# MPEGGroup/mpeg-pcc-tmc13

Measured on AMD Instinct MI355X. Metric: RAHT forward+inverse attribute-transform Mpoints/s (bit-exact vs CPU reference), higher is better.
Workload: dtype int64 (Q15 fixed point), int32 I/O; 1 GPU; subnode=1 pred=1 ext=1 qp34: RAHT forward+inverse, 1x1000000 Morton-sorted S-lidar/GPU, C=1; frames_per_gpu=1, roundtrip_decoder_equals_encoder_recon=True

## Files before the change

### mpeg-pcc-tmc13_amd/csrc/gpcc_attr_mi355.hip

```cpp
#include <hip/hip_runtime.h>

#include <algorithm>
#include <cstdio>
#include <cstdlib>
#include <dlfcn.h>
#include <cstring>
#include <atomic>
#include <deque>
#include <map>
#include <mutex>
#include <thread>
#include <string>
#include <cmath>
#include <vector>

#include "gpcc_attr_mi355.h"
#include "raht_common.hpp"
#include "raht_edges.hpp"
#include "raht_levels.hpp"
#include "raht_rdoq.hpp"
#include "raht_subnode.hpp"
#include "raht_pipe.hpp"
#include "raht_sweep.hpp"
#include "raht_tile.hpp"
// ... 960 lines not shown
    rc.state = pl.rtile_state;
    rc.c = C;
    HIP_TRY(hipMemsetAsync(pl.rtile_state, 0, ((size_t)pl.num_rtiles + 1) * sizeof(unsigned long long), st));
    HIP_TRY(hipMemsetAsync(pl.slice_l, 0xff, 2 * (size_t)s * sizeof(int32_t), st));
  }

  if (tiles) {
    lc.li = 0;
    const int cgrid = std::min(s, 2048);
    if (!encoder) {
      Timer t(ctx, "coarse_synth");
      raht_coarse_kernel<C, kCoarseDecode><<<cgrid, 1024, 0, st>>>(lc);
    } else if (pl.haar) {
      Timer t(ctx, "coarse_fused");
      raht_coarse_kernel<C, kCoarseHaar><<<cgrid, 1024, 0, st>>>(lc);
    } else {
      Timer t(ctx, "coarse_lossy");
      raht_coarse_kernel<C, kCoarseLossy><<<cgrid, 1024, 0, st>>>(lc);
    }
  }

  HIP_TRY(hipEventSynchronize(ctx->ev_stats));
  const TreeStats ts = *ctx->h_stats;
  const int first_level = std::min(nlev - 1, tiles ? ts.fine_levels : ts.max_top);

  bool piped = false;
  if (pl.pipe && first_level >= 1) {
    PipeCtx px{};
    int64_t total = 0;
    for (int li = 0; li <= first_level; li++) {
      px.uoff[li] = (int32_t)total;
      total += ts.nodes[li];
    }
    const size_t need = (size_t)total * (4 + 1 + 4 + 32 * C) + 2048;
    void* pipe_mem = nullptr;
    PoolScope pipe_pool(ctx);
    if (total * C * 16 < ((int64_t)1 << 31) && pipe_pool.take_bytes(need, &pipe_mem) == hipSuccess) {
      Arena pa;
      pa.base = (char*)pipe_mem;
      pa.cap = need;
      px.g = pa.take<uint32_t>((size_t)total * C * 4);
      px.u = pa.take<uint32_t>((size_t)total * C * 4);
      px.src = pa.take<int32_t>(total);
      px.worklist = pa.take<int32_t>(total);
      px.pocc = pa.take<uint8_t>(total);
      px.total = (int32_t)total;
      px.top = first_level;
      px.tag = 1;
      px.ticket = lc.ticket;
      HIP_TRY(hipMemsetAsync(px.g, 0, (size_t)total * C * 16, st));
      HIP_TRY(hipMemsetAsync(px.u, 0, (size_t)total * C * 16, st));
      {
        Timer t(ctx, "pipe_prepass");
        pipe_iota_kernel<<<grid_for(total, 256), 256, 0, st>>>(px.src, (int)total);
        for (int li = first_level - 1; li >= 0; li--) {
          lc.li = li;
          const int64_t parents = ts.nodes[li + 1];
          raht_pipe_prepass_kernel<C><<<(int)std::min<int64_t>((parents + 1023) / 1024, 1024), 256, 0, st>>>(lc, px);
        }
      }
      {
        Timer t(ctx, "pipe_synth");
        if (pl.f64)
          raht_pipe_synth_kernel<C, ArithF64><<<kSubGrid, 256, 0, st>>>(lc, px);
        else
          raht_pipe_synth_kernel<C><<<kSubGrid, 256, 0, st>>>(lc, px);
      }
      {
        Timer t(ctx, "pipe_leaf");
        pipe_leaf_kernel<C><<<grid_for(ts.nodes[0], 256), 256, 0, st>>>(lc, px);
      }
      piped = true;
    }
  }

  LinkSchedule links;
  auto link_prof = [&](const char* name, int li) { return Timer(ctx, li < 0 ? name : level_name(name, li)); };
  const bool use_links = pl.links && !piped && !tiles && first_level >= 1 && hp->raht_extension != 0;
  if (use_links) {
    links.tv = tv;
    links.lv = pl.lv;
    links.begin(st, ts.nodes, first_level, link_prof);
  }
  int level_from = first_level;
  static const int rec_mode = [] {
    const char* e = getenv("GPCC_REC");
    return e ? atoi(e) : 0;
  }();
  const bool ext_flag = hp->raht_extension != 0;
  const bool use_rec = pl.sub && !pl.haar && !pl.has_qp && !pl.links && !piped && rec_mode == 1;
  size_t rec_need = 0;
  if (use_rec)
// ... 5888 lines not shown
```

### mpeg-pcc-tmc13_amd/csrc/raht_levels.hpp

```cpp
#pragma once

#include "raht_common.hpp"

namespace gpcc {

enum LevelMode { kAnalyze = 0, kSynth = 1, kFused = 2, kLossySub = 3 };

constexpr uint32_t kDescNever = 0x7fffffffu;
constexpr uint32_t kDescZero = 0x80000000u;

typedef const __attribute__((address_space(4))) gpcc_raht_params* ParamsConst;

struct InterRef {
  const int64_t* pos;
  const int32_t* prefix;
  int32_t n_ref;
  int32_t lr;
  int32_t blocks;
  int32_t dual;
  int32_t filtered;
  const int32_t* tap;
  const int64_t* hkey;
  const int32_t* hfp;
  const int32_t* hlf;
  const int32_t* hsoff;
  uint32_t* idesc;
  int64_t* iptrans;
  int32_t* icoeffs;
};

enum SweepField {
  kSfW = 0, kSfCa = 1, kSfCb = 4, kSfNsq = 7, kSfNrs = 8, kSfPn = 9, kSfNbc0 = 12, kSfPk = 15, kSfPk2 = 16,
  kSfC0 = 17, kSfSlice = 18, kSweepFields = 19
};

struct SweepRec {
  int32_t* f32;
  int64_t* src;
  uint8_t* occ;
  int32_t lanes;
  int32_t rbase[kMaxLevels];
  const int32_t* worklist;
  const int32_t* work_count;
};


struct LevelCtx {
  TreeView tv;
  const gpcc_raht_params* params;
  const SliceSched* sched;
  const int32_t* attr_prefix;
  const int32_t* const* haar_lf;
  const int32_t* const* asc_qp;
  int64_t* rec[2];
  int64_t* rec_us[2];
  int32_t* nneigh[2];
  int32_t* dqp[2];
  int32_t* coeffs;
  uint32_t* desc;
  int64_t* ptrans;
  int32_t li;
  const struct SharedLut* lut;
  int32_t* worklist;
  int32_t* work_count;
  unsigned long long* scan_state;
  uint8_t* pocc;
  uint32_t* mbox;
  uint32_t mtag;
  int32_t* ticket;
  int32_t* error;
  unsigned long long* rdoq_state;
  int32_t* slice_l;
  InterRef inter;
  const int32_t* link_rec;
  const int32_t* link_lrec;
  int32_t claim_rounds;
  SweepRec brec;
};
// ... 332 lines not shown
```

### mpeg-pcc-tmc13_amd/csrc/raht_pipe.hpp

```cpp
#pragma once

#include "raht_arith.hpp"
#include "raht_subnode.hpp"

namespace gpcc {

#ifdef GPCC_PIPE_PROF
__device__ unsigned long long g_pipe_prof[32 * 8];
struct PipeProf {
  unsigned long long last = 0;
  int li = 0;
  __device__ void begin(int l) { li = l; last = __builtin_amdgcn_s_memtime(); }
  __device__ void mark(int stage, int lane)
  {
    const unsigned long long t = __builtin_amdgcn_s_memtime();
    if (lane == 0)
      atomicAdd(&g_pipe_prof[li * 8 + stage], t - last);
    last = t;
  }
  __device__ void round(int lane) { if (lane == 0) atomicAdd(&g_pipe_prof[li * 8 + 7], 1ull); }
};
#else
struct PipeProf {
  __device__ void begin(int) {}
  __device__ void mark(int, int) {}
  __device__ void round(int) {}
};
#endif

struct PipeCtx {
  int32_t* src;
  uint32_t* g;
  uint32_t* u;
  uint8_t* pocc;
  int32_t* worklist;
  int32_t uoff[kMaxLevels + 1];
  int32_t total;
  int32_t top;
  uint32_t tag;
  int32_t* ticket;
};

constexpr int32_t kPipeCopied = (int32_t)0x80000000;
constexpr int32_t kPipeIndex = 0x7fffffff;

__global__ __launch_bounds__(256) void
pipe_iota_kernel(int32_t* src, int n)
{
  for (int i = blockIdx.x * blockDim.x + threadIdx.x; i < n; i += gridDim.x * blockDim.x)
    src[i] = i;
}

template<int C>
__global__ __launch_bounds__(256) void
raht_pipe_prepass_kernel(LevelCtx ctx, PipeCtx px)
{
  __shared__ int wave_cnt[4];
  __shared__ int base_s;
  if (tree_failed(ctx.tv))
    return;
  const TreeView& tv = ctx.tv;
  const int li = ctx.li;
  const bool ext = ctx.params->raht_extension != 0;
  const int num_parents = tv.soff[li + 1][tv.num_slices];
  const int lane = lane_id(), wave = threadIdx.x >> 6;
  const int pbase = px.uoff[li + 1], cbase = px.uoff[li];
  const int64_t chunks = ((int64_t)num_parents + 255) >> 8;
  const int64_t per = (chunks + gridDim.x - 1) / gridDim.x;
  const int64_t gbeg = min((int64_t)blockIdx.x * per, chunks);
  const int64_t gend = min(gbeg + per, chunks);

  int mine = 0;
  for (int64_t chunk = gbeg; chunk < gend; chunk++) {
// ... 78 lines not shown
    int off = running;
    for (int w = 0; w < wave; w++)
      off += wave_cnt[w];
    if (real)
      px.worklist[pbase + off + __popcll(m & ((1ull << lane) - 1))] = j;
    running += wave_cnt[0] + wave_cnt[1] + wave_cnt[2] + wave_cnt[3];
  }
}

template<int C>
__global__ __launch_bounds__(256) void
pipe_leaf_kernel(LevelCtx ctx, PipeCtx px)
{
  if (tree_failed(ctx.tv))
    return;
  const TreeView& tv = ctx.tv;
  const int m = tv.soff[0][tv.num_slices];
  for (int j = blockIdx.x * blockDim.x + threadIdx.x; j < m; j += gridDim.x * blockDim.x) {
    const int s = find_slice(tv.soff[0], tv.num_slices, j);
    const SliceSched* sc = &ctx.sched[s];
    if (sc->num_unique <= 1)
      continue;
    const int64_t row = (int64_t)tv.pt_off[s] + (j - tv.soff[0][s]);
    const int from = px.src[px.uoff[0] + j] & kPipeIndex;
    const u32x4* gp = reinterpret_cast<const u32x4*>(px.g);
#pragma unroll
    for (int k = 0; k < C; k++) {
      const u32x4 gv = gp[(size_t)from * C + k];
      par2(ctx.rec, sc->final_parity)[row * C + k] = (int64_t)(((uint64_t)gv.y << 32) | gv.x);
    }
  }
}

template<int C, class A = ArithI64>
__global__ __launch_bounds__(256, C == 3 ? GPCC_SUB_SYNTH3_WAVES : 4) void
raht_pipe_synth_kernel(LevelCtx ctx, PipeCtx px)
{
  typedef typename A::T VT;
  typedef typename A::Coef VC;
  __shared__ SharedLut lut_s;
  if (tree_failed(ctx.tv))
    return;
  load_lut(&lut_s, ctx.lut);
  const SharedLut& lut = lut_s;

  const TreeView& tv = ctx.tv;
  const ParamsConst prm = (ParamsConst)ctx.params;
  const int t = threadIdx.x & 7;
  const int lane = lane_id();
  const int gbase = threadIdx.x & 56;
  const bool haar = !A::kF64 && prm->integer_haar_enable_flag != 0;
  const bool ext = A::kF64 || prm->raht_extension != 0;
  const int cls = blockIdx.x & 7;
  bool in_range = true;
  const auto grsrc = __builtin_amdgcn_make_buffer_rsrc(
    px.g, 0, (int)((size_t)px.total * C * 16), 0x00020000);
  const auto ursrc = __builtin_amdgcn_make_buffer_rsrc(
    px.u, 0, (int)((size_t)px.total * C * 16), 0x00020000);

  for (;;) {
    int tk = 0;
    if (lane == 0)
      tk = atomicAdd(&px.ticket[cls], 1);
    tk = __shfl(tk, 0);
    const int64_t ground = (int64_t)tk * 8 + cls;
    int li = -1;
    int64_t rbase = 0;
    for (int l = px.top - 1; l >= 0; l--) {
      const int64_t r = ((int64_t)ctx.work_count[l] + 7) >> 3;
      if (ground < rbase + r) {
        li = l;
        break;
      }
      rbase += r;
    }
    if (li < 0)
      break;
    if (__hip_atomic_load(ctx.error, __ATOMIC_RELAXED, __HIP_MEMORY_SCOPE_AGENT))
      break;
    PipeProf prof;
    prof.begin(li);
    prof.round(lane);
    const int num_work = ctx.work_count[li];
    const int wi = (int)((ground - rbase) * 8) + (lane >> 3);
    const bool live = wi < num_work;
    const int pbase = px.uoff[li + 1], cbase = px.uoff[li];
    const int j = live ? px.worklist[pbase + wi] : 0;
    int s = 0;
    LevelSched e;
    e.processed = 0;
    if (live) {
      s = find_slice(tv.soff[li + 1], tv.num_slices, j);
      e = ctx.sched[s].lvl[li];
    }
    const bool on = live && e.processed;
    const int sp0 = on ? tv.soff[li + 1][s] : 0;
    const int sp1 = on ? tv.soff[li + 1][s + 1] : 0;
    const int sc0 = on ? tv.soff[li][s] : 0;
    const int pt0 = on ? tv.pt_off[s] : 0;
    const int n_s = on ? tv.pt_off[s + 1] - pt0 : 0;
    const int c0 = on ? tv.fc[li + 1][j] : 0;
    const int nchild = on ? tv.fc[li + 1][j + 1] - c0 : 0;
    const int pj = j - sp0;

    const int64_t ckey = t < nchild ? tv.key[li][c0 + t] : 0;
    const uint32_t occ = group8_or(t < nchild ? 1u << (int)(ckey & 7) : 0u);
    const bool has = (occ >> t) & 1;
    const int child = c0 + popc32(occ & ((1u << t) - 1));
    int32_t w = 0;
    if (has)
      w = tv.fp[li][child + 1] - tv.fp[li][child];

    prof.mark(0, lane);
    int32_t wl[3], wr[3];
    VC ca[3], cb[3];
    int32_t cw = w;
#pragma unroll
    for (int st = 0; st < 3; st++) {
      const int bit = 1 << st;
      const int32_t pw = lane_xor8(cw, bit);
      const bool left = !(t & bit);
      wl[st] = left ? cw : pw;
      wr[st] = left ? pw : cw;
      int64_t ia = 0, ib = 0;
      if (wl[st] && wr[st]) {
        if (!haar)
          raht_coeffs(wl[st], wr[st], lut, &ia, &ib);
        cw = wl[st] + wr[st];
      } else {
        cw = left ? wl[st] + wr[st] : 0;
      }
      ca[st] = A::coef(ia);
      cb[st] = A::coef(ib);
    }

    const bool inherit_dc = !e.is_root;
    const bool pred_in_level = on && inherit_dc && prm->raht_prediction_enabled_flag != 0;
    bool enable_pred = pred_in_level;
    int neigh_count = 0;
    VT pred[C];
#pragma unroll
    for (int k = 0; k < C; k++)
      pred[k] = A::zero();
    bool want_search = false;
    if (pred_in_level) {
      if (ext && nchild == 1) {
        enable_pred = false;
        neigh_count = 19;
      } else {
        want_search = true;
      }
    }
    const int pbase_j = pbase + j;
    const int psrc_raw = (on && inherit_dc && t == 0) ? px.src[pbase_j] : 0;
    const int psrc = psrc_raw & kPipeIndex;
    int64_t own_v[C], own_us[C];
    int own_nn = 0;
    bool a1_done = false;
    {
      const bool need = on && inherit_dc && t == 0;
      u32x4 a[C], b[C];
#pragma unroll
      for (int k = 0; k < C; k++) {
        own_v[k] = own_us[k] = 0;
        a[k] = b[k] = u32x4{0, 0, 0, 0};
        if (need) {
          a[k] = __builtin_amdgcn_raw_buffer_load_b128(grsrc, (psrc * C + k) * 16, 0,  16);
          b[k] = __builtin_amdgcn_raw_buffer_load_b128(ursrc, (psrc * C + k) * 16, 0,  16);
        }
      }
      bool ok = need;
#pragma unroll
      for (int k = 0; k < C; k++)
        ok = ok && a[k].z == px.tag && b[k].z == px.tag;
      if (ok) {
#pragma unroll
        for (int k = 0; k < C; k++) {
          own_v[k] = (int64_t)(((uint64_t)a[k].y << 32) | a[k].x);
          own_us[k] = (int64_t)(((uint64_t)b[k].y << 32) | b[k].x);
        }
        own_nn = (int)a[0].w;
        a1_done = true;
      }
    }
    {
      const int early = __shfl(a1_done ? ((psrc_raw & kPipeCopied) ? 19 : own_nn) : 1 << 20, gbase);
      if (want_search && early < prm->raht_prediction_threshold0)
        want_search = false;
    }
    int pn[3] = {-1, -1, -1};
    {
      int lo[3] = {0, 0, 0}, hi[3] = {0, 0, 0}, end[3] = {0, 0, 0};
      int64_t want[3] = {0, 0, 0};
      if (want_search) {
        const int64_t cur_pos = tv.key[li + 1][j];
        const uint64_t base = morton3d_add((uint64_t)cur_pos, ~0ull);
        const int64_t range = prm->raht_prediction_search_range;
#pragma unroll
        for (int slot = 0; slot < 3; slot++) {
          const int i = 1 + t + 8 * slot;
          if (i < 19 && (occ & neigh_mask(i))) {
            const int64_t np = (int64_t)morton3d_add(base, neigh_offset(i));
            int64_t d = np - cur_pos;
            if (d >= 0) {
              d = d >= range ? range : d;
              lo[slot] = j;
              end[slot] = (d + 1 < (int64_t)(sp1 - j)) ? j + (int)(d + 1) : sp1;
            } else {
              d = (-d) >= range ? range : -d;
              end[slot] = j;
              lo[slot] = (d < (int64_t)(j - sp0)) ? j - (int)d : sp0;
            }
            hi[slot] = end[slot];
            want[slot] = np;
          }
        }
      }
      const int64_t* __restrict__ pkey = tv.key[li + 1];
      while (__any((lo[0] < hi[0]) | (lo[1] < hi[1]) | (lo[2] < hi[2]))) {
        int mid[3];
        int64_t kv[3];
#pragma unroll
        for (int slot = 0; slot < 3; slot++) {
          mid[slot] = lo[slot] + ((hi[slot] - lo[slot]) >> 1);
          kv[slot] = lo[slot] < hi[slot] ? pkey[mid[slot]] : 0;
        }
#pragma unroll
        for (int slot = 0; slot < 3; slot++) {
          if (lo[slot] < hi[slot]) {
            if (kv[slot] < want[slot])
              lo[slot] = mid[slot] + 1;
            else
              hi[slot] = mid[slot];
          }
        }
      }
#pragma unroll
      for (int slot = 0; slot < 3; slot++) {
        if (lo[slot] < end[slot] && pkey[lo[slot]] == want[slot])
          pn[slot] = lo[slot];
      }
    }

    prof.mark(1, lane);
    const uint32_t present = group8_bits(on && cw != 0) | (on ? 1u : 0u);
    const int spos = (0x74516230u >> (4 * t)) & 7;
    const uint32_t pscan = ((present >> 0) & 1) | (((present >> 4) & 1) << 1)
      | (((present >> 2) & 1) << 2) | (((present >> 1) & 1) << 3)
      | (((present >> 6) & 1) << 4) | (((present >> 5) & 1) << 5)
      | (((present >> 3) & 1) << 6) | (((present >> 7) & 1) << 7);
    const int rank = popc32(pscan & ((1u << spos) - 1));
    const bool coded = on && ((present >> t) & 1) && (t != 0 || !inherit_dc);
    const int cidx = e.coeff_base + (inherit_dc ? (c0 - sc0) - pj + rank - 1 : rank);
    const int32_t* __restrict__ cplane = ctx.coeffs + (size_t)pt0 * C + cidx;
    Quantizer qa[2] = {{1, 1}, {1, 1}};
    if (coded) {
      int ac0 = 0, ac1 = 0;
      if (e.ac_layer < prm->num_ac_qp_layers && t) {
        ac0 = prm->ac_qp_offset[e.ac_layer][t - 1][0];
        ac1 = prm->ac_qp_offset[e.ac_layer][t - 1][1];
      }
      qpset_quantizers(prm, e.qp_layer, ac0, ac1, qa);
    }
    int32_t nrm_sq_i = 0, nrm_rs_i = 0, nrm_shift = 0;
    if (!haar && w > 1) {
      nrm_sq_i = (int32_t)sqrt_weight(w, lut);
      if (w < kSmallN) {
        nrm_rs_i = lut.norm_rs[w];
      } else {
        const uint64_t w64 = (uint64_t)w;
        nrm_shift = w64 > 1024 ? ilog2_u64(w64 - 1) >> 1 : 0;
        nrm_rs_i = (int32_t)(irsqrt(w64, lut.rsqrt) >> (40 - nrm_shift - kFpFrac));
      }
    }
    const VC nrm_sq = A::coef(nrm_sq_i), nrm_rs = A::coef(nrm_rs_i);
    const typename A::Quant qaa[2] = {A::quant(qa[0]), A::quant(qa[1])};
    int32_t qc[C];
#pragma unroll
    for (int k = 0; k < C; k++)
      qc[k] = coded ? cplane[(size_t)k * n_s] : 0;

    int nsrc[3] = {0, 0, 0};
#pragma unroll
    for (int slot = 0; slot < 3; slot++)
      if (pn[slot] >= 0)
        nsrc[slot] = px.src[pbase + pn[slot]] & kPipeIndex;

    prof.mark(2, lane);
    unsigned spins = 0;
    bool failed = false;
    {
      bool need = on && inherit_dc && t == 0 && !a1_done;
      while (__any(need)) {
        u32x4 a[C], b[C];
#pragma unroll
        for (int k = 0; k < C; k++) {
          a[k] = b[k] = u32x4{0, 0, 0, 0};
          if (need) {
            a[k] = __builtin_amdgcn_raw_buffer_load_b128(grsrc, (psrc * C + k) * 16, 0,  16);
            b[k] = __builtin_amdgcn_raw_buffer_load_b128(ursrc, (psrc * C + k) * 16, 0,  16);
          }
        }
        bool ok = need;
#pragma unroll
        for (int k = 0; k < C; k++)
          ok = ok && a[k].z == px.tag && b[k].z == px.tag;
        if (ok) {
#pragma unroll
          for (int k = 0; k < C; k++) {
            own_v[k] = (int64_t)(((uint64_t)a[k].y << 32) | a[k].x);
            own_us[k] = (int64_t)(((uint64_t)b[k].y << 32) | b[k].x);
          }
          own_nn = (int)a[0].w;
          need = false;
        }
        if (!__any(ok)) {
          if (++spins > (1u << 21)) {
            failed = true;
            break;
          }
          __builtin_amdgcn_s_sleep(GPCC_SUB_SLEEP);
        }
      }
    }
    const int pneigh = __shfl((psrc_raw & kPipeCopied) ? 19 : own_nn, gbase);
    bool do_search = false;
    if (pred_in_level && !(ext && nchild == 1)) {
      if (pneigh < prm->raht_prediction_threshold0)
        enable_pred = false;
      else
        do_search = true;
    }
    if (!do_search) {
      pn[0] = pn[1] = pn[2] = -1;
    }
    {
      int found = (pn[0] >= 0) + (pn[1] >= 0) + (pn[2] >= 0);
      found = group8_sum(found);
      if (do_search) {
        neigh_count = found + 1;
        if (neigh_count < prm->raht_prediction_threshold1)
          enable_pred = false;
      }
    }
    const bool run = do_search && enable_pred;

    prof.mark(3, lane);
    int64_t nbv[3][C];
#pragma unroll
    for (int slot = 0; slot < 3; slot++)
#pragma unroll
      for (int k = 0; k < C; k++)
        nbv[slot][k] = 0;
    if (!failed) {
      uint32_t need = 0;
#pragma unroll
      for (int slot = 0; slot < 3; slot++)
        if (run && pn[slot] >= 0)
          need |= 1u << slot;
      while (__any(need != 0)) {
        u32x4 a[3][C];
#pragma unroll
        for (int slot = 0; slot < 3; slot++)
#pragma unroll
          for (int k = 0; k < C; k++) {
            a[slot][k] = u32x4{0, 0, 0, 0};
            if ((need >> slot) & 1)
              a[slot][k] = __builtin_amdgcn_raw_buffer_load_b128(
                grsrc, (nsrc[slot] * C + k) * 16, 0,  16);
          }
        bool any_ok = false;
#pragma unroll
        for (int slot = 0; slot < 3; slot++) {
          bool ok = (need >> slot) & 1;
#pragma unroll
          for (int k = 0; k < C; k++)
            ok = ok && a[slot][k].z == px.tag;
          if (ok) {
#pragma unroll
            for (int k = 0; k < C; k++)
              nbv[slot][k] = (int64_t)(((uint64_t)a[slot][k].y << 32) | a[slot][k].x);
            need &= ~(1u << slot);
            any_ok = true;
          }
        }
        if (!__any(any_ok)) {
          if (++spins > (1u << 21)) {
            failed = true;
            break;
          }
          __builtin_amdgcn_s_sleep(GPCC_SUB_SLEEP);
        }
      }
    }
    if (__any(failed)) {
      if (lane == 0)
        atomicExch(ctx.error, 1);
      break;
    }

    prof.mark(4, lane);
    VT dc[C];
#pragma unroll
    for (int k = 0; k < C; k++) {
      const int64_t val = own_us[k];
      dc[k] = A::from_i64(
        (on && inherit_dc && t == 0)
          ? (ext ? val : (val > 0 ? val << (kFpFrac - 2) : -((-val) << (kFpFrac - 2))))
          : 0);
      in_range = in_range && A::below(dc[k], A::kInvLimit);
    }

    int wsum = 0;
    VT lim_lo = A::zero(), lim_hi = A::zero();
#pragma unroll
    for (int i = 0; i < 7; i++) {
      int q;
      VT v[C];
      if (i == 0) {
        q = j;
#pragma unroll
        for (int k = 0; k < C; k++)
          v[k] = A::from_i64(shfl_i64(own_v[k], gbase));
      } else {
        q = __shfl(pn[0], gbase | (i - 1));
#pragma unroll
        for (int k = 0; k < C; k++)
          v[k] = A::from_i64(shfl_i64(nbv[0][k], gbase | (i - 1)));
      }
#pragma unroll
      for (int k = 0; k < C; k++)
        in_range = in_range && A::below(v[k], A::kRecLimit);
      if (!run || q < 0)
        continue;
      if (i) {
        if (A::muli(v[0], 10) <= lim_lo || A::muli(v[0], 10) >= lim_hi)
          continue;
      } else {
        lim_lo = A::muli(v[0], 2);
        lim_hi = A::muli(v[0], 25);
      }
      if (has && ((neigh_mask(i) >> t) & 1)) {
        const int pw = prm->pred_weight_parent[i];
        wsum += pw;
        const int mul = ext ? pw : (pw << kFpFrac);
#pragma unroll
        for (int k = 0; k < C; k++)
          pred[k] += A::muli(v[k], mul);
      }
    }

    int nb_c0[3] = {0, 0, 0};
    uint32_t nb_occ[3] = {0, 0, 0};
#pragma unroll
    for (int slot = 0; slot < 3; slot++) {
      const int i = 1 + t + 8 * slot;
      if (run && i >= 7 && i < 19 && pn[slot] >= 0) {
        const int q = pn[slot];
        if (q < j) {
          nb_c0[slot] = tv.fc[li + 1][q];
          nb_occ[slot] = px.pocc[pbase + q];
        }
      }
    }
    uint32_t pend = 0;
    int32_t nrow12[12];
    uint32_t inw = 0, wsrc_a = 0, wsrc_b = 0;
    int jg[8];
#pragma unroll
    for (int g = 0; g < 8; g++)
      jg[g] = __shfl(on ? j : -1, g << 3);
    uint32_t own = 0;
#pragma unroll
    for (int i12 = 0; i12 < 12; i12++) {
      nrow12[i12] = 0;
      const int i = 7 + i12;
      const int owner = gbase | ((i - 1) & 7);
      const int sl = (i - 1) >> 3;
      const int q = __shfl(pn[sl], owner);
      const int qc0 = __shfl(nb_c0[sl], owner);
      const uint32_t qocc = __shfl(nb_occ[sl], owner);
      VT v[C];
#pragma unroll
      for (int k = 0; k < C; k++) {
        v[k] = A::from_i64(shfl_i64(nbv[sl][k], owner));
        in_range = in_range && A::below(v[k], A::kRecLimit);
      }
      if (!run || q < 0)
        continue;
      if (A::muli(v[0], 10) <= lim_lo || A::muli(v[0], 10) >= lim_hi)
        continue;
      if (has && ((neigh_mask(i) >> t) & 1)) {
        const int sh = occu_shift(i12);
        const int cpos = i12 < 9 ? t + sh : t - sh;
        const bool child_ok = cpos >= 0 && cpos < 8 && ((qocc >> cpos) & 1);
        if (child_ok) {
          nrow12[i12] = cbase + qc0 + popc32(qocc & ((1u << cpos) - 1));
          wsum += (int)prm->pred_weight_child[i12];
          pend |= 1u << i12;
          int pg = -1;
#pragma unroll
          for (int g = 0; g < 7; g++)
            pg = q == jg[g] ? g : pg;
          if (pg >= 0) {
            own |= 1u << i12;
            if (i12 < 10)
              wsrc_a |= (uint32_t)pg << (3 * i12);
            else
              wsrc_b |= (uint32_t)pg << (3 * (i12 - 10));
          }
        } else {
          const int pwp = prm->pred_weight_parent[i];
          wsum += pwp;
          const int mul = ext ? pwp : (pwp << kFpFrac);
#pragma unroll
          for (int k = 0; k < C; k++)
            pred[k] += A::muli(v[k], mul);
        }
      }
    }
    {
      int32_t from[12];
#pragma unroll
      for (int i12 = 0; i12 < 12; i12++)
        from[i12] = ((pend >> i12) & 1) ? px.src[nrow12[i12]] : 0;
#pragma unroll
      for (int i12 = 0; i12 < 12; i12++) {
        if (!((pend >> i12) & 1))
          continue;
        const int f = from[i12] & kPipeIndex;
        if (((own >> i12) & 1) && f == nrow12[i12])
          inw |= 1u << i12;
        nrow12[i12] = f;
      }
    }
#pragma unroll
    for (int b4 = 0; b4 < 12; b4 += 4) {
      u32x4 gq[4][C];
#pragma unroll
      for (int q4 = 0; q4 < 4; q4++)
#pragma unroll
        for (int k = 0; k < C; k++) {
          gq[q4][k] = u32x4{0, 0, 0, 0};
          if (((pend & ~inw) >> (b4 + q4)) & 1)
            gq[q4][k] = __builtin_amdgcn_raw_buffer_load_b128(
              grsrc, (nrow12[b4 + q4] * C + k) * 16, 0,  16);
        }
#pragma unroll
      for (int q4 = 0; q4 < 4; q4++) {
        const int i12 = b4 + q4;
        bool ok = ((pend & ~inw) >> i12) & 1;
#pragma unroll
        for (int k = 0; k < C; k++)
          ok = ok && gq[q4][k].z == px.tag;
        if (ok) {
          const int pwc = prm->pred_weight_child[i12];
          const int mul = ext ? pwc : (pwc << kFpFrac);
#pragma unroll
          for (int k = 0; k < C; k++) {
            const VT cv = A::from_i64((int64_t)(((uint64_t)gq[q4][k].y << 32) | gq[q4][k].x));
            in_range = in_range && A::below(cv, A::kRecLimit);
            pred[k] += A::muli(cv, mul);
          }
          pend &= ~(1u << i12);
        }
      }
    }
    const VC pdiv = A::coef(pred_divisor(wsum > 0 ? wsum : 1));

    prof.mark(5, lane);
    int stage = on ? 0 : 3;
    VT pt[C];
#pragma unroll
    for (int k = 0; k < C; k++)
      pt[k] = A::zero();
    while (__any(stage != 3)) {
      bool progressed = false;
      if (__any(stage == 0 && inw)) {
#pragma unroll
        for (int i12 = 0; i12 < 12; i12++) {
          const bool mine = stage == 0 && ((inw >> i12) & 1);
          if (!__any(mine))
            continue;
          const int pg = (i12 < 10 ? wsrc_a >> (3 * i12) : wsrc_b >> (3 * (i12 - 10))) & 7;
          const int sh = occu_shift(i12);
          const int srcl = (pg << 3) | ((i12 < 9 ? t + sh : t - sh) & 7);
          const int pst = __shfl(stage, srcl);
          VT v[C];
#pragma unroll
          for (int k = 0; k < C; k++)
            v[k] = shfl_v(pt[k], srcl);
          if (mine && pst == 3) {
            const int pwc = prm->pred_weight_child[i12];
            const int mul = ext ? pwc : (pwc << kFpFrac);
#pragma unroll
            for (int k = 0; k < C; k++)
              pred[k] += A::muli(v[k], mul);
            pend &= ~(1u << i12);
            inw &= ~(1u << i12);
          }
        }
      }
      const uint32_t pm = stage == 0 ? (pend & ~inw) : 0u;
// ... 16 lines not shown
#pragma unroll
        for (int k = 0; k < C; k++)
          ok = ok && g[k].z == px.tag;
        if (ok) {
          const int mul = ext ? pwc : (pwc << kFpFrac);
#pragma unroll
          for (int k = 0; k < C; k++) {
            const VT cv = A::from_i64((int64_t)(((uint64_t)g[k].y << 32) | g[k].x));
            in_range = in_range && A::below(cv, A::kRecLimit);
            pred[k] += A::muli(cv, mul);
          }
          pend &= ~(1u << slot);
        }
      }
      const bool blocked = group8_any(stage == 0 && pend);
      const bool nready = stage == 0 && !blocked;

      if (__any(nready)) {
        progressed = true;
        VT pw_[C];
#pragma unroll
        for (int k = 0; k < C; k++)
          pw_[k] = pred[k];
        if (run && has) {
#pragma unroll
          for (int k = 0; k < C; k++) {
            pw_[k] = A::mulc(pw_[k], pdiv);
            if constexpr (!A::kF64) {
              if (haar)
                pw_[k] = (pw_[k] >> kFpFrac) << kFpFrac;
            }
          }
        }
        if (!haar && w > 1 && enable_pred) {
#pragma unroll
          for (int k = 0; k < C; k++)
            pw_[k] = A::mulc(pw_[k], nrm_sq);
        }
#pragma unroll
        for (int k = 0; k < C; k++)
          in_range = in_range && A::below(pw_[k], A::kFwdLimit);
#pragma unroll
        for (int st = 0; st < 3; st++) {
          const int bit = 1 << st;
          const bool left = !(t & bit);
          const bool both = wl[st] && wr[st];
          const bool swap = !wl[st] && wr[st];
#pragma unroll
          for (int k = 0; k < C; k++) {
            const VT own = pw_[k], oth = shfl_xor_v(own, bit);
            if (enable_pred) {
              if (both) {
                if (haar) {
                  if constexpr (!A::kF64) {
                    const int64_t hf = left ? oth - own : own - oth;
                    pw_[k] = left ? own + ((hf >> (1 + kFpFrac)) << kFpFrac) : hf;
                  }
                } else {
                  pw_[k] = left ? A::mulc(oth, cb[st]) + A::mulc(own, ca[st])
                                : A::mulc(own, ca[st]) - A::mulc(oth, cb[st]);
                }
              } else if (swap) {
                pw_[k] = oth;
              }
            }
          }
        }
// ... 22 lines not shown
          for (int k = 0; k < C; k++)
            pw_[k] = dc[k];
        }
#pragma unroll
        for (int k = 0; k < C; k++)
          in_range = in_range && A::below(pw_[k], A::kInvLimit);
#pragma unroll
        for (int st = 2; st >= 0; st--) {
          const int bit = 1 << st;
          const bool left = !(t & bit);
          const bool both = wl[st] && wr[st];
          const bool swap = !wl[st] && wr[st];
#pragma unroll
          for (int k = 0; k < C; k++) {
            const VT own = pw_[k], oth = shfl_xor_v(own, bit);
            if (both) {
              if (haar) {
                if constexpr (!A::kF64) {
                  const int64_t lf = left ? own : oth, hf = left ? oth : own;
                  const int64_t lv = lf - ((hf >> (1 + kFpFrac)) << kFpFrac);
                  pw_[k] = left ? lv : hf + lv;
                }
              } else {
                pw_[k] = left ? A::mulc(own, ca[st]) - A::mulc(oth, cb[st])
                              : A::mulc(oth, cb[st]) + A::mulc(own, ca[st]);
              }
            } else if (swap) {
              pw_[k] = oth;
            }
          }
        }
        if (can && has) {
          const uint32_t nn = (uint32_t)(inherit_dc ? neigh_count : 19);
          const int uc = cbase + child;
#pragma unroll
          for (int k = 0; k < C; k++) {
            VT v = pw_[k];
            if (!haar && w > 1)
              v = A::mulc(A::shr(v, nrm_shift), nrm_rs);
            v = ext ? v : A::round_int(v);
            pt[k] = v;
            const int64_t vi = A::to_i64(v);
            const u32x4 gr = {(uint32_t)vi, (uint32_t)((uint64_t)vi >> 32), px.tag, nn};
            __builtin_amdgcn_raw_buffer_store_b128(gr, grsrc, (uc * C + k) * 16, 0,  16);
          }
#pragma unroll
          for (int k = 0; k < C; k++) {
            const int64_t us = A::to_i64(ext ? pw_[k] : A::round_int(A::muli(pw_[k], 4)));
            const u32x4 ur = {(uint32_t)us, (uint32_t)((uint64_t)us >> 32), px.tag, 0u};
            __builtin_amdgcn_raw_buffer_store_b128(ur, ursrc, (uc * C + k) * 16, 0,  16);
          }
        }
        if (can)
          stage = 3;
      }

      if (!progressed) {
        if (++spins > (1u << 21)) {
          if (lane == 0)
            atomicExch(ctx.error, 1);
          break;
        }
        __builtin_amdgcn_s_sleep(GPCC_SUB_SLEEP);
      }
    }
    prof.mark(6, lane);
  }
  if (A::kF64 && __any(!in_range) && lane == 0)
    atomicCAS(ctx.error, 0, 3);
}

}
```

Before: 106.0 Mpoints/s.

## Precompute per-round pipe synth metadata in a separate record kernel

Adds a raht_pipe_record_kernel that, before the persistent pipelined synth kernel runs, computes each round's coefficients, normalisation factors, quantizer QPs, neighbour search results, child row sources and packed flags, and stores them in a structure-of-arrays buffer. The synth kernel then just loads these records instead of doing the Morton neighbour search, slice lookup and child resolution on its dependency-serialised critical path. This moves independent work off the latency-bound pipeline into a fully parallel pre-pass, at the cost of an extra kernel launch, a larger scratch allocation and extra memory traffic. The early-exit optimisation that skipped the search when the parent's neighbour count was already known is dropped, because the search now always runs in the pre-pass.

```diff
diff --git a/mpeg-pcc-tmc13_amd/csrc/gpcc_attr_mi355.hip b/mpeg-pcc-tmc13_amd/csrc/gpcc_attr_mi355.hip
--- a/mpeg-pcc-tmc13_amd/csrc/gpcc_attr_mi355.hip
+++ b/mpeg-pcc-tmc13_amd/csrc/gpcc_attr_mi355.hip
@@ -1016,7 +1016,11 @@
       px.uoff[li] = (int32_t)total;
       total += ts.nodes[li];
     }
-    const size_t need = (size_t)total * (4 + 1 + 4 + 32 * C) + 2048;
+    int64_t rec_rounds = 0;
+    for (int li = first_level - 1; li >= 0; li--)
+      rec_rounds += (level_max_blocks(ts.nodes, li, hp->raht_extension != 0) + 7) / 8;
+    const size_t rec_ints = (size_t)rec_rounds * 64 * kPipeFields;
+    const size_t need = (size_t)total * (4 + 1 + 4 + 32 * C) + rec_ints * 4 + 4096;
     void* pipe_mem = nullptr;
     PoolScope pipe_pool(ctx);
     if (total * C * 16 < ((int64_t)1 << 31) && pipe_pool.take_bytes(need, &pipe_mem) == hipSuccess) {
@@ -1025,6 +1029,8 @@
       pa.cap = need;
       px.g = pa.take<uint32_t>((size_t)total * C * 4);
       px.u = pa.take<uint32_t>((size_t)total * C * 4);
+      px.rec = pa.take<int32_t>(rec_ints);
+      px.rec_lanes = rec_rounds * 64;
       px.src = pa.take<int32_t>(total);
       px.worklist = pa.take<int32_t>(total);
       px.pocc = pa.take<uint8_t>(total);
@@ -1042,6 +1048,10 @@
           const int64_t parents = ts.nodes[li + 1];
           raht_pipe_prepass_kernel<C><<<(int)std::min<int64_t>((parents + 1023) / 1024, 1024), 256, 0, st>>>(lc, px);
         }
+      }
+      if (rec_rounds > 0) {
+        Timer t(ctx, "pipe_record");
+        raht_pipe_record_kernel<C><<<(int)std::min<int64_t>((rec_rounds + 3) / 4, 2048), 256, 0, st>>>(lc, px);
       }
       {
         Timer t(ctx, "pipe_synth");
diff --git a/mpeg-pcc-tmc13_amd/csrc/raht_levels.hpp b/mpeg-pcc-tmc13_amd/csrc/raht_levels.hpp
--- a/mpeg-pcc-tmc13_amd/csrc/raht_levels.hpp
+++ b/mpeg-pcc-tmc13_amd/csrc/raht_levels.hpp
@@ -44,6 +44,11 @@
   const int32_t* work_count;
 };
 
+enum PipeField {
+  kPfCa = 0, kPfCb = 3, kPfNsq = 6, kPfNrs = 7, kPfNorm = 8, kPfPk = 9, kPfNsrc = 10, kPfChild = 13, kPfUc = 25,
+  kPfCidx = 26, kPfQp = 27, kPfMisc = 28, kPipeFields = 29
+};
+constexpr int32_t kPfNone = -1, kPfParent = -2, kPfInWave = 1 << 30, kPfIndex = (1 << 27) - 1;
 
 struct LevelCtx {
   TreeView tv;
diff --git a/mpeg-pcc-tmc13_amd/csrc/raht_pipe.hpp b/mpeg-pcc-tmc13_amd/csrc/raht_pipe.hpp
--- a/mpeg-pcc-tmc13_amd/csrc/raht_pipe.hpp
+++ b/mpeg-pcc-tmc13_amd/csrc/raht_pipe.hpp
@@ -39,6 +39,8 @@
   int32_t top;
   uint32_t tag;
   int32_t* ticket;
+  int32_t* rec;
+  int64_t rec_lanes;
 };
 
 constexpr int32_t kPipeCopied = (int32_t)0x80000000;
@@ -183,63 +185,55 @@
   }
 }
 
-template<int C, class A = ArithI64>
-__global__ __launch_bounds__(256, C == 3 ? GPCC_SUB_SYNTH3_WAVES : 4) void
-raht_pipe_synth_kernel(LevelCtx ctx, PipeCtx px)
+__device__ __forceinline__ int
+pipe_round_level(const int32_t* __restrict__ work_count, int top, int64_t ground, int64_t* rbase_out)
 {
-  typedef typename A::T VT;
-  typedef typename A::Coef VC;
+  int64_t rbase = 0;
+  for (int l = top - 1; l >= 0; l--) {
+    const int64_t r = ((int64_t)work_count[l] + 7) >> 3;
+    if (ground < rbase + r) {
+      *rbase_out = rbase;
+      return l;
+    }
+    rbase += r;
+  }
+  return -1;
+}
+
+template<int C>
+__global__ __launch_bounds__(256) void
+raht_pipe_record_kernel(LevelCtx ctx, PipeCtx px)
+{
   __shared__ SharedLut lut_s;
   if (tree_failed(ctx.tv))
     return;
   load_lut(&lut_s, ctx.lut);
   const SharedLut& lut = lut_s;
-
   const TreeView& tv = ctx.tv;
   const ParamsConst prm = (ParamsConst)ctx.params;
   const int t = threadIdx.x & 7;
   const int lane = lane_id();
   const int gbase = threadIdx.x & 56;
-  const bool haar = !A::kF64 && prm->integer_haar_enable_flag != 0;
-  const bool ext = A::kF64 || prm->raht_extension != 0;
-  const int cls = blockIdx.x & 7;
-  bool in_range = true;
-  const auto grsrc = __builtin_amdgcn_make_buffer_rsrc(
-    px.g, 0, (int)((size_t)px.total * C * 16), 0x00020000);
-  const auto ursrc = __builtin_amdgcn_make_buffer_rsrc(
-    px.u, 0, (int)((size_t)px.total * C * 16), 0x00020000);
-
-  for (;;) {
-    int tk = 0;
-    if (lane == 0)
-      tk = atomicAdd(&px.ticket[cls], 1);
-    tk = __shfl(tk, 0);
-    const int64_t ground = (int64_t)tk * 8 + cls;
-    int li = -1;
+  const bool haar = prm->integer_haar_enable_flag != 0;
+  const bool ext = prm->raht_extension != 0;
+  const size_t ln = (size_t)px.rec_lanes;
+  for (int64_t ground = (int64_t)blockIdx.x * 4 + (threadIdx.x >> 6);; ground += (int64_t)gridDim.x * 4) {
     int64_t rbase = 0;
-    for (int l = px.top - 1; l >= 0; l--) {
-      const int64_t r = ((int64_t)ctx.work_count[l] + 7) >> 3;
-      if (ground < rbase + r) {
-        li = l;
-        break;
-      }
-      rbase += r;
-    }
+    const int li = pipe_round_level(ctx.work_count, px.top, ground, &rbase);
     if (li < 0)
       break;
-    if (__hip_atomic_load(ctx.error, __ATOMIC_RELAXED, __HIP_MEMORY_SCOPE_AGENT))
+    if ((ground + 1) * 64 > px.rec_lanes) {
+      if (lane == 0)
+        atomicExch(ctx.error, 1);
       break;
-    PipeProf prof;
-    prof.begin(li);
-    prof.round(lane);
+    }
     const int num_work = ctx.work_count[li];
     const int wi = (int)((ground - rbase) * 8) + (lane >> 3);
     const bool live = wi < num_work;
     const int pbase = px.uoff[li + 1], cbase = px.uoff[li];
     const int j = live ? px.worklist[pbase + wi] : 0;
     int s = 0;
-    LevelSched e;
-    e.processed = 0;
+    LevelSched e{};
     if (live) {
       s = find_slice(tv.soff[li + 1], tv.num_slices, j);
       e = ctx.sched[s].lvl[li];
@@ -262,88 +256,38 @@
     if (has)
       w = tv.fp[li][child + 1] - tv.fp[li][child];
 
-    prof.mark(0, lane);
-    int32_t wl[3], wr[3];
-    VC ca[3], cb[3];
+    int32_t ia3[3], ib3[3];
+    uint32_t bothm = 0, swapm = 0;
     int32_t cw = w;
 #pragma unroll
     for (int st = 0; st < 3; st++) {
       const int bit = 1 << st;
       const int32_t pw = lane_xor8(cw, bit);
       const bool left = !(t & bit);
-      wl[st] = left ? cw : pw;
-      wr[st] = left ? pw : cw;
+      const int32_t wl = left ? cw : pw, wr = left ? pw : cw;
       int64_t ia = 0, ib = 0;
-      if (wl[st] && wr[st]) {
+      if (wl && wr) {
         if (!haar)
-          raht_coeffs(wl[st], wr[st], lut, &ia, &ib);
-        cw = wl[st] + wr[st];
+          raht_coeffs(wl, wr, lut, &ia, &ib);
+        cw = wl + wr;
       } else {
-        cw = left ? wl[st] + wr[st] : 0;
-      }
-      ca[st] = A::coef(ia);
-      cb[st] = A::coef(ib);
+        cw = left ? wl + wr : 0;
+      }
+      ia3[st] = (int32_t)ia;
+      ib3[st] = (int32_t)ib;
+      bothm |= (wl && wr) ? 1u << st : 0u;
+      swapm |= (!wl && wr) ? 1u << st : 0u;
     }
 
     const bool inherit_dc = !e.is_root;
     const bool pred_in_level = on && inherit_dc && prm->raht_prediction_enabled_flag != 0;
-    bool enable_pred = pred_in_level;
-    int neigh_count = 0;
-    VT pred[C];
-#pragma unroll
-    for (int k = 0; k < C; k++)
-      pred[k] = A::zero();
-    bool want_search = false;
-    if (pred_in_level) {
-      if (ext && nchild == 1) {
-        enable_pred = false;
-        neigh_count = 19;
-      } else {
-        want_search = true;
-      }
-    }
-    const int pbase_j = pbase + j;
-    const int psrc_raw = (on && inherit_dc && t == 0) ? px.src[pbase_j] : 0;
-    const int psrc = psrc_raw & kPipeIndex;
-    int64_t own_v[C], own_us[C];
-    int own_nn = 0;
-    bool a1_done = false;
-    {
-      const bool need = on && inherit_dc && t == 0;
-      u32x4 a[C], b[C];
-#pragma unroll
-      for (int k = 0; k < C; k++) {
-        own_v[k] = own_us[k] = 0;
-        a[k] = b[k] = u32x4{0, 0, 0, 0};
-        if (need) {
-          a[k] = __builtin_amdgcn_raw_buffer_load_b128(grsrc, (psrc * C + k) * 16, 0,  16);
-          b[k] = __builtin_amdgcn_raw_buffer_load_b128(ursrc, (psrc * C + k) * 16, 0,  16);
-        }
-      }
-      bool ok = need;
-#pragma unroll
-      for (int k = 0; k < C; k++)
-        ok = ok && a[k].z == px.tag && b[k].z == px.tag;
-      if (ok) {
-#pragma unroll
-        for (int k = 0; k < C; k++) {
-          own_v[k] = (int64_t)(((uint64_t)a[k].y << 32) | a[k].x);
-          own_us[k] = (int64_t)(((uint64_t)b[k].y << 32) | b[k].x);
-        }
-        own_nn = (int)a[0].w;
-        a1_done = true;
-      }
-    }
-    {
-      const int early = __shfl(a1_done ? ((psrc_raw & kPipeCopied) ? 19 : own_nn) : 1 << 20, gbase);
-      if (want_search && early < prm->raht_prediction_threshold0)
-        want_search = false;
-    }
+    const bool single = pred_in_level && ext && nchild == 1;
+    const bool search = pred_in_level && !single;
     int pn[3] = {-1, -1, -1};
     {
       int lo[3] = {0, 0, 0}, hi[3] = {0, 0, 0}, end[3] = {0, 0, 0};
       int64_t want[3] = {0, 0, 0};
-      if (want_search) {
+      if (search) {
         const int64_t cur_pos = tv.key[li + 1][j];
         const uint64_t base = morton3d_add((uint64_t)cur_pos, ~0ull);
         const int64_t range = prm->raht_prediction_search_range;
@@ -392,8 +336,8 @@
           pn[slot] = lo[slot];
       }
     }
-
-    prof.mark(1, lane);
+    const int found = group8_sum((pn[0] >= 0) + (pn[1] >= 0) + (pn[2] >= 0));
+
     const uint32_t present = group8_bits(on && cw != 0) | (on ? 1u : 0u);
     const int spos = (0x74516230u >> (4 * t)) & 7;
     const uint32_t pscan = ((present >> 0) & 1) | (((present >> 4) & 1) << 1)
@@ -403,15 +347,17 @@
     const int rank = popc32(pscan & ((1u << spos) - 1));
     const bool coded = on && ((present >> t) & 1) && (t != 0 || !inherit_dc);
     const int cidx = e.coeff_base + (inherit_dc ? (c0 - sc0) - pj + rank - 1 : rank);
-    const int32_t* __restrict__ cplane = ctx.coeffs + (size_t)pt0 * C + cidx;
-    Quantizer qa[2] = {{1, 1}, {1, 1}};
+    int32_t qp2 = 0;
     if (coded) {
       int ac0 = 0, ac1 = 0;
       if (e.ac_layer < prm->num_ac_qp_layers && t) {
         ac0 = prm->ac_qp_offset[e.ac_layer][t - 1][0];
         ac1 = prm->ac_qp_offset[e.ac_layer][t - 1][1];
       }
-      qpset_quantizers(prm, e.qp_layer, ac0, ac1, qa);
+      const int qp0 = clip(prm->layer_qp[e.qp_layer][0] + ac0, 4, prm->max_qp);
+      const int qp1 = clip(prm->layer_qp[e.qp_layer][1] + ac1 + qp0, 4, prm->max_qp);
+      qp2 = (int32_t)((uint32_t)((qp0 + prm->fixed_point_qp_offset) & 0xffff)
+                      | (uint32_t)(qp1 + prm->fixed_point_qp_offset) << 16);
     }
     int32_t nrm_sq_i = 0, nrm_rs_i = 0, nrm_shift = 0;
     if (!haar && w > 1) {
@@ -424,24 +370,192 @@
         nrm_rs_i = (int32_t)(irsqrt(w64, lut.rsqrt) >> (40 - nrm_shift - kFpFrac));
       }
     }
-    const VC nrm_sq = A::coef(nrm_sq_i), nrm_rs = A::coef(nrm_rs_i);
-    const typename A::Quant qaa[2] = {A::quant(qa[0]), A::quant(qa[1])};
+
+    const int32_t psrc_raw = (on && inherit_dc && t == 0) ? px.src[pbase + j] : 0;
+    int32_t nsrc[3];
+#pragma unroll
+    for (int slot = 0; slot < 3; slot++)
+      nsrc[slot] = pn[slot] >= 0 ? (px.src[pbase + pn[slot]] & kPipeIndex) : -1;
+
+    int nb_c0[3] = {0, 0, 0};
+    uint32_t nb_occ[3] = {0, 0, 0};
+#pragma unroll
+    for (int slot = 0; slot < 3; slot++) {
+      const int i = 1 + t + 8 * slot;
+      if (i >= 7 && i < 19 && pn[slot] >= 0) {
+        const int q = pn[slot];
+        if (q < j) {
+          nb_c0[slot] = tv.fc[li + 1][q];
+          nb_occ[slot] = px.pocc[pbase + q];
+        }
+      }
+    }
+    int jg[8];
+#pragma unroll
+    for (int g = 0; g < 8; g++)
+      jg[g] = __shfl(on ? j : -1, g << 3);
+    int32_t ch[12];
+#pragma unroll
+    for (int i12 = 0; i12 < 12; i12++) {
+      const int i = 7 + i12;
+      const int owner = gbase | ((i - 1) & 7);
+      const int sl = (i - 1) >> 3;
+      const int q = __shfl(pn[sl], owner);
+      const int qc0 = __shfl(nb_c0[sl], owner);
+      const uint32_t qocc = __shfl(nb_occ[sl], owner);
+      ch[i12] = kPfNone;
+      if (q >= 0 && has && ((neigh_mask(i) >> t) & 1)) {
+        const int sh = occu_shift(i12);
+        const int cpos = i12 < 9 ? t + sh : t - sh;
+        const bool child_ok = cpos >= 0 && cpos < 8 && ((qocc >> cpos) & 1);
+        if (child_ok) {
+          const int nrow = cbase + qc0 + popc32(qocc & ((1u << cpos) - 1));
+          const int f = px.src[nrow] & kPipeIndex;
+          int pg = -1;
+#pragma unroll
+          for (int g = 0; g < 7; g++)
+            pg = q == jg[g] ? g : pg;
+          ch[i12] = (pg >= 0 && f == nrow) ? (f | kPfInWave | pg << 27) : f;
+        } else {
+          ch[i12] = kPfParent;
+        }
+      }
+    }
+
+    int32_t* __restrict__ f = px.rec + (size_t)ground * 64 + lane;
+#pragma unroll
+    for (int st = 0; st < 3; st++) {
+      f[(kPfCa + st) * ln] = ia3[st];
+      f[(kPfCb + st) * ln] = ib3[st];
+      f[(kPfNsrc + st) * ln] = nsrc[st];
+    }
+    f[kPfNsq * ln] = nrm_sq_i;
+    f[kPfNrs * ln] = nrm_rs_i;
+    f[kPfNorm * ln] = nrm_shift | ((!haar && w > 1) ? 1 << 8 : 0);
+    f[kPfPk * ln] = (int32_t)(occ | present << 8 | (uint32_t)found << 16 | bothm << 21 | swapm << 24
+                              | (on ? 1u << 27 : 0u) | ((on && inherit_dc) ? 1u << 28 : 0u)
+                              | (search ? 1u << 29 : 0u) | (single ? 1u << 30 : 0u));
+#pragma unroll
+    for (int i12 = 0; i12 < 12; i12++)
+      f[(kPfChild + i12) * ln] = ch[i12];
+    f[kPfUc * ln] = has ? cbase + child : -1;
+    f[kPfCidx * ln] = coded ? pt0 * C + cidx : -1;
+    f[kPfQp * ln] = qp2;
+    f[kPfMisc * ln] = t == 0 ? psrc_raw : (t == 1 ? n_s : 0);
+  }
+}
+
+template<int C, class A = ArithI64>
+__global__ __launch_bounds__(256, C == 3 ? GPCC_SUB_SYNTH3_WAVES : 4) void
+raht_pipe_synth_kernel(LevelCtx ctx, PipeCtx px)
+{
+  typedef typename A::T VT;
+  typedef typename A::Coef VC;
+  __shared__ SharedLut lut_s;
+  if (tree_failed(ctx.tv))
+    return;
+  load_lut(&lut_s, ctx.lut);
+  const SharedLut& lut = lut_s;
+
+  const TreeView& tv = ctx.tv;
+  const ParamsConst prm = (ParamsConst)ctx.params;
+  const int t = threadIdx.x & 7;
+  const int lane = lane_id();
+  const int gbase = threadIdx.x & 56;
+  const bool haar = !A::kF64 && prm->integer_haar_enable_flag != 0;
+  const bool ext = A::kF64 || prm->raht_extension != 0;
+  const int cls = blockIdx.x & 7;
+  bool in_range = true;
+  const auto grsrc = __builtin_amdgcn_make_buffer_rsrc(
+    px.g, 0, (int)((size_t)px.total * C * 16), 0x00020000);
+  const auto ursrc = __builtin_amdgcn_make_buffer_rsrc(
+    px.u, 0, (int)((size_t)px.total * C * 16), 0x00020000);
+
+  for (;;) {
+    int tk = 0;
+    if (lane == 0)
+      tk = atomicAdd(&px.ticket[cls], 1);
+    tk = __shfl(tk, 0);
+    const int64_t ground = (int64_t)tk * 8 + cls;
+    int64_t rbase = 0;
+    const int li = pipe_round_level(ctx.work_count, px.top, ground, &rbase);
+    if (li < 0)
+      break;
+    if (__hip_atomic_load(ctx.error, __ATOMIC_RELAXED, __HIP_MEMORY_SCOPE_AGENT))
+      break;
+    if ((ground + 1) * 64 > px.rec_lanes) {
+      if (lane == 0)
+        atomicExch(ctx.error, 1);
+      break;
+    }
+    PipeProf prof;
+    prof.begin(li);
+    prof.round(lane);
+
+    const size_t rln = (size_t)px.rec_lanes;
+    const int32_t* __restrict__ rf = px.rec + (size_t)ground * 64 + lane;
+    const uint32_t pk = (uint32_t)rf[kPfPk * rln];
+    const int32_t misc = rf[kPfMisc * rln];
+    int32_t nsrc[3], ch[12];
+    VC ca[3], cb[3];
+    int32_t wl[3], wr[3];
+#pragma unroll
+    for (int slot = 0; slot < 3; slot++)
+      nsrc[slot] = rf[(kPfNsrc + slot) * rln];
+#pragma unroll
+    for (int st = 0; st < 3; st++) {
+      const bool both = (pk >> (21 + st)) & 1u, swap = (pk >> (24 + st)) & 1u;
+      wl[st] = swap ? 0 : 1;
+      wr[st] = (both || swap) ? 1 : 0;
+      ca[st] = A::coef(rf[(kPfCa + st) * rln]);
+      cb[st] = A::coef(rf[(kPfCb + st) * rln]);
+    }
+#pragma unroll
+    for (int i12 = 0; i12 < 12; i12++)
+      ch[i12] = rf[(kPfChild + i12) * rln];
+    const int32_t uc = rf[kPfUc * rln];
+    const int32_t cidx = rf[kPfCidx * rln];
+    const int32_t qp2 = rf[kPfQp * rln];
+    const int32_t norm = rf[kPfNorm * rln];
+    const VC nrm_sq = A::coef(rf[kPfNsq * rln]), nrm_rs = A::coef(rf[kPfNrs * rln]);
+    const int nrm_shift = norm & 0xff;
+    const bool normalise = (norm >> 8) & 1;
+    const bool on = (pk >> 27) & 1u;
+    const bool inherit_dc = (pk >> 28) & 1u;
+    const bool search = (pk >> 29) & 1u, single = (pk >> 30) & 1u;
+    const bool has = (pk >> t) & 1u;
+    const bool coded = cidx >= 0;
+    const int psrc_raw = t == 0 ? misc : 0;
+    const int psrc = psrc_raw & kPipeIndex;
+    const int found = (int)((pk >> 16) & 31u);
+
+    prof.mark(0, lane);
+    const size_t n_s = (size_t)__shfl(misc, gbase | 1);
+    const typename A::Quant qaa[2] = {
+      A::quant(coded ? make_quantizer((int16_t)(qp2 & 0xffff)) : Quantizer{1, 1}),
+      A::quant(coded ? make_quantizer(qp2 >> 16) : Quantizer{1, 1})};
     int32_t qc[C];
 #pragma unroll
     for (int k = 0; k < C; k++)
-      qc[k] = coded ? cplane[(size_t)k * n_s] : 0;
-
-    int nsrc[3] = {0, 0, 0};
-#pragma unroll
-    for (int slot = 0; slot < 3; slot++)
-      if (pn[slot] >= 0)
-        nsrc[slot] = px.src[pbase + pn[slot]] & kPipeIndex;
-
-    prof.mark(2, lane);
+      qc[k] = coded ? ctx.coeffs[(size_t)cidx + (size_t)k * n_s] : 0;
+
+    bool enable_pred = search;
+    int neigh_count = single ? 19 : 0;
+    VT pred[C];
+#pragma unroll
+    for (int k = 0; k < C; k++)
+      pred[k] = A::zero();
+    int64_t own_v[C], own_us[C];
+#pragma unroll
+    for (int k = 0; k < C; k++)
+      own_v[k] = own_us[k] = 0;
+    int own_nn = 0;
+
+    prof.mark(1, lane);
     unsigned spins = 0;
     bool failed = false;
     {
-      bool need = on && inherit_dc && t == 0 && !a1_done;
+      bool need = on && inherit_dc && t == 0;
       while (__any(need)) {
         u32x4 a[C], b[C];
 #pragma unroll
@@ -476,27 +590,22 @@
     }
     const int pneigh = __shfl((psrc_raw & kPipeCopied) ? 19 : own_nn, gbase);
     bool do_search = false;
-    if (pred_in_level && !(ext && nchild == 1)) {
+    if (search) {
       if (pneigh < prm->raht_prediction_threshold0)
         enable_pred = false;
       else
         do_search = true;
     }
     if (!do_search) {
-      pn[0] = pn[1] = pn[2] = -1;
-    }
-    {
-      int found = (pn[0] >= 0) + (pn[1] >= 0) + (pn[2] >= 0);
-      found = group8_sum(found);
-      if (do_search) {
-        neigh_count = found + 1;
-        if (neigh_count < prm->raht_prediction_threshold1)
-          enable_pred = false;
-      }
+      nsrc[0] = nsrc[1] = nsrc[2] = -1;
+    } else {
+      neigh_count = found + 1;
+      if (neigh_count < prm->raht_prediction_threshold1)
+        enable_pred = false;
     }
     const bool run = do_search && enable_pred;
 
-    prof.mark(3, lane);
+    prof.mark(2, lane);
     int64_t nbv[3][C];
 #pragma unroll
     for (int slot = 0; slot < 3; slot++)
@@ -507,7 +616,7 @@
       uint32_t need = 0;
 #pragma unroll
       for (int slot = 0; slot < 3; slot++)
-        if (run && pn[slot] >= 0)
+        if (run && nsrc[slot] >= 0)
           need |= 1u << slot;
       while (__any(need != 0)) {
         u32x4 a[3][C];
@@ -550,7 +659,7 @@
       break;
     }
 
-    prof.mark(4, lane);
+    prof.mark(3, lane);
     VT dc[C];
 #pragma unroll
     for (int k = 0; k < C; k++) {
@@ -569,12 +678,12 @@
       int q;
       VT v[C];
       if (i == 0) {
-        q = j;
+        q = 0;
 #pragma unroll
         for (int k = 0; k < C; k++)
           v[k] = A::from_i64(shfl_i64(own_v[k], gbase));
       } else {
-        q = __shfl(pn[0], gbase | (i - 1));
+        q = __shfl(nsrc[0], gbase | (i - 1));
 #pragma unroll
         for (int k = 0; k < C; k++)
           v[k] = A::from_i64(shfl_i64(nbv[0][k], gbase | (i - 1)));
@@ -601,88 +710,45 @@
       }
     }
 
-    int nb_c0[3] = {0, 0, 0};
-    uint32_t nb_occ[3] = {0, 0, 0};
-#pragma unroll
-    for (int slot = 0; slot < 3; slot++) {
-      const int i = 1 + t + 8 * slot;
-      if (run && i >= 7 && i < 19 && pn[slot] >= 0) {
-        const int q = pn[slot];
-        if (q < j) {
-          nb_c0[slot] = tv.fc[li + 1][q];
-          nb_occ[slot] = px.pocc[pbase + q];
-        }
-      }
-    }
     uint32_t pend = 0;
     int32_t nrow12[12];
     uint32_t inw = 0, wsrc_a = 0, wsrc_b = 0;
-    int jg[8];
-#pragma unroll
-    for (int g = 0; g < 8; g++)
-      jg[g] = __shfl(on ? j : -1, g << 3);
-    uint32_t own = 0;
 #pragma unroll
     for (int i12 = 0; i12 < 12; i12++) {
       nrow12[i12] = 0;
       const int i = 7 + i12;
       const int owner = gbase | ((i - 1) & 7);
       const int sl = (i - 1) >> 3;
-      const int q = __shfl(pn[sl], owner);
-      const int qc0 = __shfl(nb_c0[sl], owner);
-      const uint32_t qocc = __shfl(nb_occ[sl], owner);
       VT v[C];
 #pragma unroll
       for (int k = 0; k < C; k++) {
         v[k] = A::from_i64(shfl_i64(nbv[sl][k], owner));
         in_range = in_range && A::below(v[k], A::kRecLimit);
       }
-      if (!run || q < 0)
+      const int32_t term = ch[i12];
+      if (!run || term == kPfNone)
         continue;
       if (A::muli(v[0], 10) <= lim_lo || A::muli(v[0], 10) >= lim_hi)
         continue;
-      if (has && ((neigh_mask(i) >> t) & 1)) {
-        const int sh = occu_shift(i12);
-        const int cpos = i12 < 9 ? t + sh : t - sh;
-        const bool child_ok = cpos >= 0 && cpos < 8 && ((qocc >> cpos) & 1);
-        if (child_ok) {
-          nrow12[i12] = cbase + qc0 + popc32(qocc & ((1u << cpos) - 1));
-          wsum += (int)prm->pred_weight_child[i12];
-          pend |= 1u << i12;
-          int pg = -1;
-#pragma unroll
-          for (int g = 0; g < 7; g++)
-            pg = q == jg[g] ? g : pg;
-          if (pg >= 0) {
-            own |= 1u << i12;
-            if (i12 < 10)
-              wsrc_a |= (uint32_t)pg << (3 * i12);
-            else
-              wsrc_b |= (uint32_t)pg << (3 * (i12 - 10));
-          }
-        } else {
-          const int pwp = prm->pred_weight_parent[i];
-          wsum += pwp;
-          const int mul = ext ? pwp : (pwp << kFpFrac);
-#pragma unroll
-          for (int k = 0; k < C; k++)
-            pred[k] += A::muli(v[k], mul);
-        }
-      }
-    }
-    {
-      int32_t from[12];
-#pragma unroll
-      for (int i12 = 0; i12 < 12; i12++)
-        from[i12] = ((pend >> i12) & 1) ? px.src[nrow12[i12]] : 0;
-#pragma unroll
-      for (int i12 = 0; i12 < 12; i12++) {
-        if (!((pend >> i12) & 1))
-          continue;
-        const int f = from[i12] & kPipeIndex;
-        if (((own >> i12) & 1) && f == nrow12[i12])
+      if (term != kPfParent) {
+        nrow12[i12] = term & kPfIndex;
+        wsum += (int)prm->pred_weight_child[i12];
+        pend |= 1u << i12;
+        if (term & kPfInWave) {
+          const uint32_t pg = ((uint32_t)term >> 27) & 7u;
           inw |= 1u << i12;
-        nrow12[i12] = f;
+          if (i12 < 10)
+            wsrc_a |= pg << (3 * i12);
+          else
+            wsrc_b |= pg << (3 * (i12 - 10));
+        }
+      } else {
+        const int pwp = prm->pred_weight_parent[i];
+        wsum += pwp;
+        const int mul = ext ? pwp : (pwp << kFpFrac);
+#pragma unroll
+        for (int k = 0; k < C; k++)
+          pred[k] += A::muli(v[k], mul);
       }
     }
 #pragma unroll
@@ -719,7 +785,7 @@
     }
     const VC pdiv = A::coef(pred_divisor(wsum > 0 ? wsum : 1));
 
-    prof.mark(5, lane);
+    prof.mark(4, lane);
     int stage = on ? 0 : 3;
     VT pt[C];
 #pragma unroll
@@ -802,7 +868,7 @@
             }
           }
         }
-        if (!haar && w > 1 && enable_pred) {
+        if (normalise && enable_pred) {
 #pragma unroll
           for (int k = 0; k < C; k++)
             pw_[k] = A::mulc(pw_[k], nrm_sq);
@@ -891,11 +957,10 @@
         }
         if (can && has) {
           const uint32_t nn = (uint32_t)(inherit_dc ? neigh_count : 19);
-          const int uc = cbase + child;
 #pragma unroll
           for (int k = 0; k < C; k++) {
             VT v = pw_[k];
-            if (!haar && w > 1)
+            if (normalise)
               v = A::mulc(A::shr(v, nrm_shift), nrm_rs);
             v = ext ? v : A::round_int(v);
             pt[k] = v;
@@ -923,7 +988,7 @@
         __builtin_amdgcn_s_sleep(GPCC_SUB_SLEEP);
       }
     }
-    prof.mark(6, lane);
+    prof.mark(5, lane);
   }
   if (A::kF64 && __any(!in_range) && lane == 0)
     atomicCAS(ctx.error, 0, 3);
```

Result: no change. 106.0 Mpoints/s, median of 3 (+0.0%).
